# werner-duvaud/muzero-general

Measured on NVIDIA B200. Metric: self-play env-steps/sec, higher is better.
Workload: dtype f32 nets + f64 tree statistics

## Files before the change

### muzero_general_b200/csrc/fc_search.cu

```cuda
#include "fc_net.cuh"
#include "tree.cuh"
#include "kernels.h"

#include <stdlib.h>

namespace mz {

struct GameSmem {
    int vsum, mval, root_prior, visit, expansion, reward, prior, path, path_reward, hidden, act, bytes;
};

__host__ __device__ inline GameSmem game_smem_layout(int N, int A, int E, int maxw, bool keep_hidden) {
    GameSmem L;
    const int S = (N + 1) * A;
    const int Epad = (E + 3) & ~3;
    int off = 0;
    auto take = [&](int bytes) { int o = off; off = (off + bytes + 15) & ~15; return o; };
    L.vsum = take(S * 8);
    L.mval = take(S * 8);
    L.root_prior = take(A * 8);
    L.visit = take(S * 4);
    L.expansion = take(S * 4);
    L.reward = take(S * 4);
    L.prior = take(S * 4);
    L.path = take((N + 2) * 4);
    L.path_reward = take((N + 2) * 4);
    L.hidden = take((keep_hidden ? (N + 1) * Epad : 0) * 4);
    L.act = take(9 * maxw * 4);
    off += 16;
    L.bytes = off;
    return L;
}

template <int G, bool kTeacher, typename SH>
__global__ void __launch_bounds__(kFcMaxThreads) fc_search_kernel(const __grid_constant__ FcSearchArgs a) {
    extern __shared__ __align__(16) unsigned char smem[];
    const int N = a.N, A = a.A;
    double* s_pbc = reinterpret_cast<double*>(smem);
    double* s_sqrt = s_pbc + (N + 2);
    float* s_blob = reinterpret_cast<float*>(s_sqrt + (N + 2));
    for (int i = threadIdx.x; i < N + 2; i += blockDim.x) { s_pbc[i] = a.pbc[i]; s_sqrt[i] = a.sqrtn[i]; }
    if (!kTeacher)
        for (int i = threadIdx.x; i < a.net.blob_floats; i += blockDim.x) s_blob[i] = a.blob[i];
    __syncthreads();

    const int shared_bytes = ((2 * (N + 2) * 8 + (kTeacher ? 0 : a.net.blob_floats) * 4) + 15) & ~15;
    const GameSmem L = game_smem_layout(N, A, a.net.E, a.net.maxw, !kTeacher);
    const int groups_per_cta = blockDim.x / G;
    const int gi = threadIdx.x / G;
    const int lane = LaneGroup<G>::lane();
    unsigned char* mine = smem + shared_bytes + (size_t)gi * L.bytes;

    TreeConst c;
    c.A = A; c.N = N; c.P = a.P; c.discount = a.discount; c.noise_frac = a.noise_frac; c.noise_alpha = a.noise_alpha; c.seed = a.seed;
    c.pbc = s_pbc; c.sqrtn = s_sqrt; c.ucb = a.ucb;

    GameTree t;
    t.vsum = reinterpret_cast<double*>(mine + L.vsum);
    t.mval = reinterpret_cast<double*>(mine + L.mval);
    t.root_prior = reinterpret_cast<double*>(mine + L.root_prior);
    t.visit = reinterpret_cast<int*>(mine + L.visit);
    t.expansion = reinterpret_cast<int*>(mine + L.expansion);
    t.reward = reinterpret_cast<float*>(mine + L.reward);
    t.prior = reinterpret_cast<float*>(mine + L.prior);
    t.path = reinterpret_cast<int*>(mine + L.path);
    t.path_reward = reinterpret_cast<float*>(mine + L.path_reward);
    float* s_hidden = reinterpret_cast<float*>(mine + L.hidden);
    float* s_act = reinterpret_cast<float*>(mine + L.act);
    const int E = a.net.E, F = a.net.F, S = a.net.S, maxw = a.net.maxw;
    const int Epad = (E + 3) & ~3;
    float* s0 = s_act;
    float* s1 = s_act + maxw;
    float* s2 = s_act + 2 * maxw;
    float* const hb[3][2] = {{s_act + 3 * maxw, s_act + 4 * maxw}, {s_act + 5 * maxw, s_act + 6 * maxw},
                             {s_act + 7 * maxw, s_act + 8 * maxw}};
    const bool fused_heads = (a.net.rew.n == a.net.pol.n) && (a.net.pol.n == a.net.val.n);

    for (int g = blockIdx.x * groups_per_cta + gi; g < a.n_games; g += gridDim.x * groups_per_cta) {
        const int64_t game_id = a.game_id ? a.game_id[g] : (int64_t)g;
        const int move = a.move_index ? a.move_index[g] : 0;
        const int to_play0 = a.to_play ? a.to_play[g] : 0;
        const int first_index = a.first_index ? a.first_index[g] : -1;
        unsigned legal = 0;
        for (int k = 0; k < A; ++k) legal |= (a.legal_mask == nullptr || a.legal_mask[(size_t)g * A + k]) ? (1u << k) : 0u;
        t.legal = legal;
        (void)to_play0;

        float root_value, root_reward, logit = 0.0f;
        if (kTeacher) {
            root_value = a.teacher.root_value[g];
            root_reward = a.teacher.root_reward[g];
        } else {
            load_vector<G>(a.obs + (size_t)g * a.net.obs_elems, s1, a.net.obs_elems);
            float* raw = mlp_forward<G>(a.net.rep, s_blob, s1, s0, s1, s2);
            rescale_unit_range<G>(raw, s_hidden, E);
            float* pol = mlp_forward<G>(a.net.pol, s_blob, s_hidden, s0, s1, s2);
            logit = (lane < A) ? pol[lane] : 0.0f;
            LaneGroup<G>::sync();
            float* val = mlp_forward<G>(a.net.val, s_blob, s_hidden, s0, s1, s2);
            root_value = support_to_scalar_group<G>(val, S);
            LaneGroup<G>::sync();
            root_reward = inverse_value_transform(0.0f);
        }
        float prior;
        if (kTeacher) prior = (lane < A) ? a.teacher.root_priors[(size_t)g * A + lane] : 0.0f;
        else prior = group_softmax_masked<G>(logit, lane < A && ((legal >> lane) & 1u));
        if (a.trace.root_priors_raw && lane < A) a.trace.root_priors_raw[(size_t)g * A + lane] = ((legal >> lane) & 1u) ? prior : 0.0f;
        if (a.trace.root_reward && lane == 0) a.trace.root_reward[g] = root_reward;
        tree_init_root<G>(c, t, prior, root_reward,
                          (a.add_noise && a.noise) ? a.noise + (size_t)g * A : nullptr, a.add_noise && !a.noise,
                          game_id, move, a.trace.noise ? a.trace.noise + (size_t)g * A : nullptr);

        int max_depth = 0;
        for (int sim = 0; sim < N; ++sim) {
            const Leaf leaf = tree_select<G>(c, t, sim, game_id, move, first_index);
            float value, reward;
            if (kTeacher) {
                value = a.teacher.value[(size_t)g * N + sim];
                reward = a.teacher.reward[(size_t)g * N + sim];
                prior = (lane < A) ? a.teacher.priors[((size_t)g * N + sim) * A + lane] : 0.0f;
            } else {
                const float* h = s_hidden + (size_t)leaf.parent_exp * Epad;
                float* hn = s_hidden + (size_t)t.n_expanded * Epad;
                if constexpr (SH::kEnabled) {
                    fc_recurrent_fixed<G, SH>(a.net, s_blob, h, leaf.action, hn, s0, s1, hb[0][0], hb[1][0], hb[2][0], logit, value, reward);
                } else {
                float* raw = mlp_forward<G>(a.net.dyn, s_blob, h, s0, s1, s2, leaf.action);
                if (fused_heads) {
                    rescale_unit_range<G>(raw, hn, E);
                    const MlpDesc* const ds[3] = {&a.net.rew, &a.net.pol, &a.net.val};
                    const float* const xs[3] = {raw, hn, hn};
                    float* outs[3];
                    mlp_forward_multi<G, 3>(ds, s_blob, xs, hb, outs);
                    logit = (lane < A) ? outs[1][lane] : 0.0f;
                    support_to_scalar_group2<G>(outs[2], outs[0], S, value, reward);
                    LaneGroup<G>::sync();
                } else {
                    float* rl = mlp_forward<G>(a.net.rew, s_blob, raw, s0, s1, nullptr);
                    reward = support_to_scalar_group<G>(rl, S);
                    LaneGroup<G>::sync();
                    rescale_unit_range<G>(raw, hn, E);
                    float* pol = mlp_forward<G>(a.net.pol, s_blob, hn, s0, s1, s2);
                    logit = (lane < A) ? pol[lane] : 0.0f;
                    LaneGroup<G>::sync();
                    float* vl = mlp_forward<G>(a.net.val, s_blob, hn, s0, s1, s2);
                    value = support_to_scalar_group<G>(vl, S);
                    LaneGroup<G>::sync();
                }
                }
                if constexpr (SH::kEnabled) prior = group_softmax_masked_w<G, pow2_ceil_c(SH::A)>(logit, lane < A);
                else prior = group_softmax_masked<G>(logit, lane < A);
            }
            if (a.trace.depth) {
                const size_t ti = (size_t)g * N + sim;
                if (lane == 0) { a.trace.depth[ti] = leaf.depth; a.trace.value[ti] = value; a.trace.reward[ti] = reward; }
                if (lane < A) a.trace.priors[ti * A + lane] = prior;
                for (int j = lane; j < leaf.depth && j < a.trace.max_depth; j += G)
                    a.trace.actions[ti * a.trace.max_depth + j] = (uint8_t)(t.path[j + 1] % A);
            }
            tree_expand<G>(c, t, leaf, reward, prior);
            tree_backup<G>(c, t, leaf, value);
            max_depth = max(max_depth, leaf.depth);
        }

        if (lane < A) {
            const bool ok = (legal >> lane) & 1u;
            if (a.visit_counts) a.visit_counts[(size_t)g * A + lane] = ok ? t.visit[lane] : 0;
            if (a.root_priors) a.root_priors[(size_t)g * A + lane] = t.root_prior[lane];
        }
        if (lane == 0) {
            if (a.root_value) a.root_value[g] = (t.root_visit == 0) ? 0.0 : __ddiv_rn(t.root_vsum, (double)t.root_visit);
            if (a.root_predicted_value) a.root_predicted_value[g] = root_value;
            if (a.max_tree_depth) a.max_tree_depth[g] = max_depth;
            if (a.tie_count) a.tie_count[g] = t.ties;
            if (a.value_range) { a.value_range[2 * g] = t.lo; a.value_range[2 * g + 1] = t.hi; }
        }
        if (a.pool.visit) {
            const int slots = (N + 1) * A;
            const size_t pb = (size_t)g * slots;
            for (int s = lane; s < t.n_expanded * A; s += G) {
                a.pool.visit[pb + s] = t.visit[s];
                a.pool.vsum[pb + s] = t.vsum[s];
                a.pool.reward[pb + s] = t.reward[s];
                a.pool.prior[pb + s] = t.prior[s];
                a.pool.expansion[pb + s] = t.expansion[s];
            }
            if (lane < A) a.pool.root_prior[(size_t)g * A + lane] = t.root_prior[lane];
            if (!kTeacher && a.pool.hidden)
                for (int i = lane; i < t.n_expanded * E; i += G)
                    a.pool.hidden[(size_t)g * (N + 1) * E + i] = s_hidden[(i / E) * Epad + (i % E)];
            if (lane == 0) {
                a.pool.root_visit[g] = t.root_visit;
                a.pool.root_vsum[g] = t.root_vsum;
                a.pool.n_expanded[g] = t.n_expanded;
            }
        }
        LaneGroup<G>::sync();
    }
    (void)F;
}

template <int G, bool T, typename SH>
static cudaError_t launch_one(const FcSearchArgs& a, int sm_count, size_t smem_cap, cudaStream_t stream, FcLaunchInfo* info) {
    const GameSmem L = game_smem_layout(a.N, a.A, a.net.E, a.net.maxw, !T);
    const size_t shared_bytes = ((2 * (size_t)(a.N + 2) * 8 + (T ? 0 : (size_t)a.net.blob_floats) * 4) + 15) & ~(size_t)15;
    const int threads = a.threads;
    const int groups = threads / G;
    if (groups < 1) return cudaErrorInvalidValue;
    const size_t smem = shared_bytes + (size_t)groups * L.bytes;
    if (smem > smem_cap) return cudaErrorInvalidConfiguration;
    auto kern = fc_search_kernel<G, T, SH>;
    cudaError_t err = cudaFuncSetAttribute(kern, cudaFuncAttributeMaxDynamicSharedMemorySize, (int)smem);
    if (err != cudaSuccess) return err;
    int per_sm = 0;
    err = cudaOccupancyMaxActiveBlocksPerMultiprocessor(&per_sm, kern, threads, smem);
    if (err != cudaSuccess) return err;
    if (per_sm < 1) return cudaErrorInvalidConfiguration;
    const int want = (a.n_games + groups - 1) / groups;
    const int grid = want < per_sm * sm_count ? want : per_sm * sm_count;
    if (info) { info->grid = grid; info->block = threads; info->smem = smem; info->ctas_per_sm = per_sm; info->group = G; }
    kern<<<grid, threads, smem, stream>>>(a);
    return cudaGetLastError();
}

using CartPoleShape = FcFixedShape<8, 16, 10, 2>;

cudaError_t launch_fc_search(const FcSearchArgs& a, int group, bool teacher, int sm_count, size_t smem_cap,
                             cudaStream_t stream, FcLaunchInfo* info) {
    const char* generic = getenv("MZ_FC_GENERIC");
    if (!teacher && !(generic && generic[0] == '1') && fc_matches_fixed<CartPoleShape>(a.net)) {
        if (group == 16) return launch_one<16, false, CartPoleShape>(a, sm_count, smem_cap, stream, info);
        if (group == 32) return launch_one<32, false, CartPoleShape>(a, sm_count, smem_cap, stream, info);
    }
#define MZ_CASE(GG)                                                                                     \
    case GG:                                                                                            \
        return teacher ? launch_one<GG, true, FcGenericShape>(a, sm_count, smem_cap, stream, info)      \
                       : launch_one<GG, false, FcGenericShape>(a, sm_count, smem_cap, stream, info);
    switch (group) {
        MZ_CASE(4)
        MZ_CASE(8)
        MZ_CASE(16)
        MZ_CASE(32)
    }
#undef MZ_CASE
    return cudaErrorInvalidValue;
}

size_t fc_search_smem_bytes(const FcSearchArgs& a, int group, bool teacher) {
    const GameSmem L = game_smem_layout(a.N, a.A, a.net.E, a.net.maxw, !teacher);
    const size_t shared_bytes = ((2 * (size_t)(a.N + 2) * 8 + (teacher ? 0 : (size_t)a.net.blob_floats) * 4) + 15) & ~(size_t)15;
    return shared_bytes + (size_t)(a.threads / group) * L.bytes;
}

}
```

### muzero_general_b200/csrc/kernels.h

```cpp
#pragma once
#include <cuda_runtime.h>
#include <stddef.h>
#include <stdint.h>

#include "../../include/mzb200.h"
#include "fc_net.cuh"

namespace mz {

constexpr int kFcThreads = 128;
constexpr int kFcMaxThreads = 128;

struct NodePool {
    int* visit;
    double* vsum;
    double* mval;
    float* reward;
    float* prior;
    int* expansion;
    double* root_prior;
    float* hidden;
    int* root_visit;
    double* root_vsum;
    float* root_reward;
    double* range;
    int* n_expanded;
    int* ties;
    int* max_depth;
    unsigned* legal;
    int* path;
    float* path_reward;
    int* leaf_depth;
    int* leaf_parent;
    int* leaf_action;
    int* leaf_slot;
    float* net_value;
    float* net_reward;
    float* net_policy;
};

struct DevTeacher { const float *root_value, *root_reward, *root_priors, *value, *reward, *priors; };
struct DevTrace {
    int max_depth;
    int* depth; uint8_t* actions; float *value, *reward, *priors, *root_priors_raw, *root_reward;
    double* noise;
};

struct FcSearchArgs {
    int n_games, N, A, P;
    int threads;
    double discount, noise_frac, noise_alpha;
    uint64_t seed;
    const double* pbc;
    const double* sqrtn;
    const double* ucb;
    FcNet net;
    const float* blob;
    const float* obs;
    const uint8_t* legal_mask;
    const int32_t* to_play;
    int add_noise;
    const double* noise;
    const int32_t* first_index;
    const int64_t* game_id;
    const int32_t* move_index;
    int32_t* visit_counts;
    double* root_value;
    float* root_predicted_value;
    int32_t* max_tree_depth;
    int32_t* tie_count;
    double* root_priors;
    double* value_range;
    DevTeacher teacher;
    DevTrace trace;
    NodePool pool;
};

struct FcInferArgs {
    int n, recurrent;
    FcNet net;
    const float* blob;
    const float* in;
    const int32_t* action;
    const int32_t* gather_parent;
    float* pool_hidden;
    int pool_stride, out_slot;
    float *value_logits, *reward_logits, *policy_logits, *hidden, *value, *reward;
};
cudaError_t launch_fc_inference(const FcInferArgs& a, int group, int sm_count, cudaStream_t stream);

struct FcLaunchInfo { int grid, block, ctas_per_sm, group; size_t smem; };

cudaError_t launch_fc_search(const FcSearchArgs& a, int group, bool teacher, int sm_count, size_t smem_cap,
                             cudaStream_t stream, FcLaunchInfo* info);
size_t fc_search_smem_bytes(const FcSearchArgs& a, int group, bool teacher);

}
```

### muzero_general_b200/csrc/tree.cuh

```cuda
#pragma once
#include "common.cuh"

namespace mz {

struct TreeConst {
    int A;
    int N;
    int P;
    double discount;
    double noise_frac;
    double noise_alpha;
    uint64_t seed;
    const double* pbc;
    const double* sqrtn;
    const double* ucb;
};

struct GameTree {
    int* visit;
    double* vsum;
    double* mval;
    float* reward;
    float* prior;
    int* expansion;
    double* root_prior;
    int* path;
    float* path_reward;
    int root_visit;
    double root_vsum;
    float root_reward;
    double lo, hi;
    unsigned legal;
    int n_expanded;
    int ties;
};

struct Leaf {
    int depth;
    int parent_exp;
    int action;
    int slot;
};

MZ_DEVINL double value_range_normalize(double v, double lo, double hi) {
    if (hi > lo) {
        const double d = __dsub_rn(v, lo);
        const double q = __ddiv_rn(d == 0.0 ? 1.0 : d, __dsub_rn(hi, lo));
        return d == 0.0 ? 0.0 : q;
    }
    return v;
}

MZ_DEVINL int nth_set_bit(unsigned m, int n) { return (int)__fns(m, 0, n + 1); }

template <int G>
MZ_DEVINL float group_softmax_masked(float logit, bool valid) {
    const float m = group_max_f32<G>(valid ? logit : -INFINITY);
    const float e = valid ? expf(logit - m) : 0.0f;
    const float s = group_sum_f32<G>(e);
    return div_pos_or_zero(e, s);
}

template <int G, int W>
MZ_DEVINL float group_softmax_masked_w(float logit, bool valid) {
    const float m = group_max_f32_w<G, W>(valid ? logit : -INFINITY);
    const float e = valid ? expf(logit - m) : 0.0f;
    const float s = group_sum_f32_w<G, W>(e);
    return div_pos_or_zero(e, s);
}

template <int G>
MZ_DEVINL void tree_init_root(const TreeConst& c, GameTree& t, float prior_f32, float root_reward,
                              const double* noise , bool generate_noise = false,
                              int64_t game_id = 0, int move = 0, double* noise_out = nullptr) {
    const int k = LaneGroup<G>::lane();
    const bool legal = (k < c.A) && ((t.legal >> k) & 1u);
    double nz = 0.0;
    bool have_noise = false;
    if (noise != nullptr) {
        nz = legal ? noise[k] : 0.0;
        have_noise = true;
    } else if (generate_noise) {
        const double gm = legal ? philox_gamma(c.seed, game_id, move, k, c.noise_alpha) : 0.0;
        double sum = gm;
        const unsigned m = LaneGroup<G>::mask();
        for (int off = G >> 1; off > 0; off >>= 1) sum += shfl_xor_f64(m, sum, off, G);
        nz = gm / sum;
        have_noise = true;
    }
    if (noise_out && k < c.A) noise_out[k] = nz;
    if (k < c.A) {
        double p = (double)prior_f32;
        if (legal && have_noise) {
            p = __dadd_rn(__dmul_rn(p, __dsub_rn(1.0, c.noise_frac)), __dmul_rn(nz, c.noise_frac));
        }
        t.root_prior[k] = legal ? p : 0.0;
        t.visit[k] = 0;
        t.vsum[k] = 0.0;
        t.reward[k] = 0.0f;
        t.prior[k] = legal ? prior_f32 : 0.0f;
        t.expansion[k] = -1;
    }
    t.root_visit = 0;
    t.root_vsum = 0.0;
    t.root_reward = root_reward;
    t.lo = INFINITY;
    t.hi = -INFINITY;
    t.n_expanded = 1;
    t.ties = 0;
    LaneGroup<G>::sync();
}

template <int G, bool kPool = false>
MZ_DEVINL Leaf tree_select(const TreeConst& c, GameTree& t, int sim, int64_t game_id, int move, int first_index) {
    const int k = LaneGroup<G>::lane();
    const int width = pow2_ceil(c.A);
    int e = 0;
    int n_parent = t.root_visit;
    int depth = 0;
    Leaf leaf;
    if (k == 0) { t.path[0] = -1; t.path_reward[0] = t.root_reward; }
    while (true) {
        const int base = e * c.A;
        const bool valid = (k < c.A) && (e != 0 || ((t.legal >> k) & 1u));
        double score = -INFINITY;
        int nc = 0, child_exp_k = -1;
        float reward_k = 0.0f;
        if (valid) {
            nc = t.visit[base + k];
            child_exp_k = t.expansion[base + k];
            const double pr = (e == 0) ? t.root_prior[k] : (double)t.prior[base + k];
            double mv = 0.0, tab_pbc = 0.0, tab_sqrt = 0.0;
            if (kPool) {
                reward_k = t.reward[base + k];
                mv = t.mval[base + k];
                tab_pbc = __ldg(c.pbc + n_parent);
                tab_sqrt = __ldg(c.sqrtn + n_parent);
                if (child_exp_k >= 0) {
                    const int nb = child_exp_k * c.A;
                    prefetch_l1(t.visit + nb); prefetch_l1(t.expansion + nb); prefetch_l1(t.prior + nb);
                    prefetch_l1(t.reward + nb); prefetch_l1(t.mval + nb);
                    prefetch_l1(t.mval + nb + c.A - 1);
                }
            }
            double pbc;
            if (kPool) {
                pbc = __dmul_rn(tab_pbc, __ddiv_rn(tab_sqrt, (double)(nc + 1)));
            } else if (c.ucb) {
                pbc = __ldg(c.ucb + n_parent * (c.N + 2) + nc);
            } else {
                const double q = __ddiv_rn(c.sqrtn[n_parent], (double)(nc + 1));
                pbc = __dmul_rn(c.pbc[n_parent], q);
            }
            score = __dmul_rn(pbc, pr);
            if (nc > 0) {
                if (!kPool) reward_k = t.reward[base + k];
                const double v = value_range_normalize(kPool ? mv : t.mval[base + k], t.lo, t.hi);
                score = __dadd_rn(score, v);
            } else {
                reward_k = 0.0f;
                score = __dadd_rn(score, 0.0);
            }
        }
        const double best = group_max_f64<G>(score, width > G ? G : width);
        const unsigned tied = LaneGroup<G>::ballot(valid && score == best);
        const int n_tied = __popc(tied);
        int pick;
        if (n_tied <= 1) {
            pick = max(__ffs(tied) - 1, 0);
        } else {
            int idx;
            if (sim == 0 && depth == 0 && first_index >= 0) {
                idx = first_index < n_tied ? first_index : n_tied - 1;
            } else {
                idx = philox_tie_index(c.seed, game_id, move, sim, depth, n_tied);
                if (!(sim == 0 && depth == 0)) t.ties += 1;
            }
            pick = nth_set_bit(tied, idx);
        }
        const int slot = base + pick;
        depth += 1;
        const int child_exp = LaneGroup<G>::bcast(child_exp_k, pick);
        const int child_visits = LaneGroup<G>::bcast(nc, pick);
        if (k == pick) { t.path[depth] = slot; t.path_reward[depth] = reward_k; }
        if (child_exp < 0) {
            leaf.depth = depth;
            leaf.parent_exp = e;
            leaf.action = pick;
            leaf.slot = slot;
            break;
        }
        n_parent = child_visits;
        e = child_exp;
    }
    LaneGroup<G>::sync();
    return leaf;
}

template <int G>
MZ_DEVINL int tree_expand(const TreeConst& c, GameTree& t, const Leaf& leaf, float reward, float prior_f32) {
    const int k = LaneGroup<G>::lane();
    const int e = t.n_expanded;
    if (k == 0) {
        t.expansion[leaf.slot] = e;
        t.reward[leaf.slot] = reward;
        t.path_reward[leaf.depth] = reward;
    }
    if (k < c.A) {
        const int s = e * c.A + k;
        t.visit[s] = 0;
        t.vsum[s] = 0.0;
        t.reward[s] = 0.0f;
        t.prior[s] = prior_f32;
        t.expansion[s] = -1;
    }
    t.n_expanded = e + 1;
    LaneGroup<G>::sync();
    return e;
}

template <int G>
MZ_DEVINL void tree_backup(const TreeConst& c, GameTree& t, const Leaf& leaf, float leaf_value) {
    const int k = LaneGroup<G>::lane();
    const int L = leaf.depth;
    double lo = INFINITY, hi = -INFINITY;
    double v = (double)leaf_value;
    double root_vsum = t.root_vsum;
    const bool packed = (L < G);
    int my_slot = -1;
    float my_reward = 0.0f;
    if (packed && k <= L) { my_slot = t.path[k]; my_reward = t.path_reward[k]; }
    if (packed) {
        double myv = 0.0;
        for (int j = L; j >= 0; --j) {
            const double r = (double)LaneGroup<G>::bcast(my_reward, j);
            const bool same = (c.P == 1) || (((L - j) & 1) == 0);
            if (j == k) myv = v;
            const double rr = (c.P == 1) ? r : (same ? -r : r);
            v = __dadd_rn(rr, __dmul_rn(c.discount, v));
        }
        if (k <= L) {
            const bool same = (c.P == 1) || (((L - k) & 1) == 0);
            const double add = same ? myv : -myv;
            double q;
            if (k == 0) {
                root_vsum = __dadd_rn(t.root_vsum, add);
                q = __ddiv_rn(root_vsum, (double)(t.root_visit + 1));
            } else {
                const double s = __dadd_rn(t.vsum[my_slot], add);
                const int n = t.visit[my_slot] + 1;
                t.vsum[my_slot] = s;
                t.visit[my_slot] = n;
                q = __ddiv_rn(s, (double)n);
            }
            const double m = __dadd_rn((double)my_reward, __dmul_rn(c.discount, (c.P == 1) ? q : -q));
            if (k > 0) t.mval[my_slot] = m;
            lo = m;
            hi = m;
        }
    } else {
    for (int j = L; j >= 0; --j) {
        const int slot = t.path[j];
        const float rf = t.path_reward[j];
        const double r = (double)rf;
        const bool same = (c.P == 1) || (((L - j) & 1) == 0);
        if ((j % G) == k) {
            const double add = same ? v : -v;
            double q;
            if (j == 0) {
                root_vsum = __dadd_rn(t.root_vsum, add);
                q = __ddiv_rn(root_vsum, (double)(t.root_visit + 1));
            } else {
                const double s = __dadd_rn(t.vsum[slot], add);
                const int n = t.visit[slot] + 1;
                t.vsum[slot] = s;
                t.visit[slot] = n;
                q = __ddiv_rn(s, (double)n);
            }
            const double m = __dadd_rn(r, __dmul_rn(c.discount, (c.P == 1) ? q : -q));
            if (j > 0) t.mval[slot] = m;
            lo = fmin(lo, m);
            hi = fmax(hi, m);
        }
        const double rr = (c.P == 1) ? r : (same ? -r : r);
        v = __dadd_rn(rr, __dmul_rn(c.discount, v));
    }
    }
    const int width = (L + 1 >= G) ? G : pow2_ceil(L + 1);
    const unsigned gm = LaneGroup<G>::mask();
    if (width >= 2) {
        const int half = width >> 1;
        const bool up = (k & half) != 0;
        const double got = shfl_xor_f64(gm, up ? lo : hi, half, G);
        double val = up ? fmax(hi, got) : fmin(lo, got);
        for (int off = half >> 1; off > 0; off >>= 1) {
            const double r = shfl_xor_f64(gm, val, off, G);
            val = up ? fmax(val, r) : fmin(val, r);
        }
        lo = shfl_f64(gm, val, 0, G);
        hi = shfl_f64(gm, val, half, G);
    } else {
        lo = shfl_f64(gm, lo, 0, G);
        hi = shfl_f64(gm, hi, 0, G);
    }
    root_vsum = shfl_f64(gm, root_vsum, 0, G);
    t.root_vsum = root_vsum;
    t.root_visit += 1;
    t.lo = fmin(t.lo, lo);
    t.hi = fmax(t.hi, hi);
    LaneGroup<G>::sync();
}

}
```

Baseline: 10.57 million.

## Add multi-level lookahead tree selection using idle lanes for binary-action games

Adds a tree-selection routine for games with at most two actions. The spare lanes of each lane group evaluate UCB scores for several tree levels at once, so one round of shuffles and ballots descends up to K levels instead of one. This cuts the number of serial, synchronised descent steps per simulation. In exchange, each lane does redundant pointer-chasing loads through shared memory, and the tie-breaking and path bookkeeping become more intricate. It is enabled by default when A<=2 and can be turned off with an environment variable.

```diff
diff --git a/muzero_general_b200/csrc/fc_search.cu b/muzero_general_b200/csrc/fc_search.cu
--- a/muzero_general_b200/csrc/fc_search.cu
+++ b/muzero_general_b200/csrc/fc_search.cu
@@ -113,7 +113,13 @@
 
         int max_depth = 0;
         for (int sim = 0; sim < N; ++sim) {
-            const Leaf leaf = tree_select<G>(c, t, sim, game_id, move, first_index);
+            Leaf leaf;
+            if constexpr (lookahead_levels<G>() >= 2) {
+                if (a.lookahead) leaf = tree_select_lookahead<G>(c, t, sim, game_id, move, first_index);
+                else leaf = tree_select<G>(c, t, sim, game_id, move, first_index);
+            } else {
+                leaf = tree_select<G>(c, t, sim, game_id, move, first_index);
+            }
             float value, reward;
             if (kTeacher) {
                 value = a.teacher.value[(size_t)g * N + sim];
@@ -225,8 +231,11 @@
 
 using CartPoleShape = FcFixedShape<8, 16, 10, 2>;
 
-cudaError_t launch_fc_search(const FcSearchArgs& a, int group, bool teacher, int sm_count, size_t smem_cap,
+cudaError_t launch_fc_search(const FcSearchArgs& args, int group, bool teacher, int sm_count, size_t smem_cap,
                              cudaStream_t stream, FcLaunchInfo* info) {
+    FcSearchArgs a = args;
+    const char* la = getenv("MZ_FC_LOOKAHEAD");
+    a.lookahead = (a.A <= 2 && !(la && la[0] == '0')) ? 1 : 0;
     const char* generic = getenv("MZ_FC_GENERIC");
     if (!teacher && !(generic && generic[0] == '1') && fc_matches_fixed<CartPoleShape>(a.net)) {
         if (group == 16) return launch_one<16, false, CartPoleShape>(a, sm_count, smem_cap, stream, info);
diff --git a/muzero_general_b200/csrc/kernels.h b/muzero_general_b200/csrc/kernels.h
--- a/muzero_general_b200/csrc/kernels.h
+++ b/muzero_general_b200/csrc/kernels.h
@@ -74,6 +74,7 @@
     DevTeacher teacher;
     DevTrace trace;
     NodePool pool;
+    int lookahead;
 };
 
 struct FcInferArgs {
diff --git a/muzero_general_b200/csrc/tree.cuh b/muzero_general_b200/csrc/tree.cuh
--- a/muzero_general_b200/csrc/tree.cuh
+++ b/muzero_general_b200/csrc/tree.cuh
@@ -198,6 +198,108 @@
 }
 
 template <int G>
+constexpr int lookahead_levels() { return G >= 32 ? 4 : G >= 16 ? 3 : G >= 8 ? 2 : 1; }
+
+template <int G>
+MZ_DEVINL Leaf tree_select_lookahead(const TreeConst& c, GameTree& t, int sim, int64_t game_id, int move, int first_index) {
+    constexpr int K = lookahead_levels<G>();
+    static_assert(K >= 2, "lookahead needs at least two levels per round");
+    const int k = LaneGroup<G>::lane();
+    const int A = c.A;
+    int e = 0;
+    int n_parent = t.root_visit;
+    int depth = 0;
+    Leaf leaf;
+    if (k == 0) { t.path[0] = -1; t.path_reward[0] = t.root_reward; }
+    while (true) {
+        int kr = k;
+        asm volatile("" : "+r"(kr));
+        const int j = kr + 2 - (2 << (30 - __clz(kr + 2)));
+        const int lvl = (kr < (2 << K) - 2 && (A == 2 || j == 0)) ? 30 - __clz(kr + 2) : K;
+        int node = lvl < K ? e : -1, np = n_parent;
+#pragma unroll
+        for (int i = 0; i < K - 1; ++i) {
+            if (i < lvl && node >= 0) {
+                const int s = node * A + ((j >> (lvl - i)) & 1);
+                np = t.visit[s];
+                node = t.expansion[s];
+            }
+        }
+        const int a_own = j & 1;
+        const int slot_k = node * A + a_own;
+        const bool root_level = (node == 0);
+        const bool valid = node >= 0 && (!root_level || ((t.legal >> a_own) & 1u));
+        double score = -INFINITY;
+        int nc = 0, child_exp_k = -1;
+        float reward_k = 0.0f;
+        if (valid) {
+            nc = t.visit[slot_k];
+            child_exp_k = t.expansion[slot_k];
+            const double pr = root_level ? t.root_prior[a_own] : (double)t.prior[slot_k];
+            double pbc;
+            if (c.ucb) {
+                pbc = __ldg(c.ucb + np * (c.N + 2) + nc);
+            } else {
+                const double q = __ddiv_rn(c.sqrtn[np], (double)(nc + 1));
+                pbc = __dmul_rn(c.pbc[np], q);
+            }
+            score = __dmul_rn(pbc, pr);
+            if (nc > 0) {
+                reward_k = t.reward[slot_k];
+                const double v = value_range_normalize(t.mval[slot_k], t.lo, t.hi);
+                score = __dadd_rn(score, v);
+            } else {
+                score = __dadd_rn(score, 0.0);
+            }
+        }
+        const double best = fmax(score, shfl_xor_f64(LaneGroup<G>::mask(), score, 1, G));
+        const unsigned tied = LaneGroup<G>::ballot(valid && score == best);
+        const unsigned expanded = LaneGroup<G>::ballot(child_exp_k >= 0);
+        int pl = 0;
+        int p = 0;
+#pragma unroll
+        for (int l = 0; l < K; ++l) {
+            const int pair = (2 << l) - 2 + 2 * p;
+            const unsigned tl = (tied >> pair) & 3u;
+            const int n_tied = __popc(tl);
+            int pick;
+            if (n_tied <= 1) {
+                pick = max(__ffs(tl) - 1, 0);
+            } else {
+                int idx;
+                const int d = depth + l;
+                if (sim == 0 && d == 0 && first_index >= 0) {
+                    idx = first_index < n_tied ? first_index : n_tied - 1;
+                } else {
+                    idx = philox_tie_index(c.seed, game_id, move, sim, d, n_tied);
+                    if (!(sim == 0 && d == 0)) t.ties += 1;
+                }
+                pick = nth_set_bit(tl, idx);
+            }
+            pl = pair + pick;
+            if (k == pl) { t.path[depth + l + 1] = slot_k; t.path_reward[depth + l + 1] = reward_k; }
+            if (!((expanded >> pl) & 1u)) break;
+            p = 2 * p + pick;
+        }
+        const int child_exp = LaneGroup<G>::bcast(child_exp_k, pl);
+        const int child_visits = LaneGroup<G>::bcast(nc, pl);
+        const int slot = LaneGroup<G>::bcast(slot_k, pl);
+        depth += 31 - __clz(pl + 2);
+        if (child_exp < 0) {
+            leaf.depth = depth;
+            leaf.parent_exp = (A == 2) ? (slot >> 1) : slot;
+            leaf.action = (A == 2) ? (slot & 1) : 0;
+            leaf.slot = slot;
+            break;
+        }
+        n_parent = child_visits;
+        e = child_exp;
+    }
+    LaneGroup<G>::sync();
+    return leaf;
+}
+
+template <int G>
 MZ_DEVINL int tree_expand(const TreeConst& c, GameTree& t, const Leaf& leaf, float reward, float prior_f32) {
     const int k = LaneGroup<G>::lane();
     const int e = t.n_expanded;
```

Measured after the change: 11.18 million (median of 6 runs). +5.8%, better.
